# Spijkervet/Context-Aware-Sequential-Recommendation

Hardware: AMD Instinct MI355X
Metric: user-sequences/sec (fwd+bwd) (higher is better)
Workload: dtype f32 (bf16x3 split MFMA in attention); 1 GPU; ml-1m-shaped synthetic (6040 users, 3416 items), cast_1 maxlen=200 hidden_units=50 num_blocks=2 num_heads=1 dropout=0.20, batch 128/GPU (global 128), fwd+bwd+dense TF-Adam per step; parallelism=dp1, hip_graph=True, steps_per_graph_launch=4, attn_precision=bf16x3

## Files before the change

### context-aware-sequential-recommendation_amd/csrc/cr_adam.hip

```cpp
#include <math.h>
#include <stdlib.h>
#include <string.h>

#include "cr_common.hpp"
#include "cr_tgrad.hpp"

int tg_unit_grid(const cr_tgrad_desc* d);

#define ADAM_COLS 256
#define ADAM_WAVES 16
typedef float f4a __attribute__((ext_vector_type(4), aligned(4)));
__device__ __forceinline__ float slab_sum256(const float* slabs, int n_slabs, int n_dense, int j0, float (*part)[ADAM_COLS]) {
    const int lane = threadIdx.x & 63, w = threadIdx.x >> 6;
    const int j = j0 + 4 * lane;
    f4a acc = (f4a){0.f, 0.f, 0.f, 0.f};
    if (j + 3 < n_dense) {
        for (int s0 = w; s0 < n_slabs; s0 += 16 * ADAM_WAVES) {
            f4a v[16];
            int cnt = 0;
#pragma unroll
            for (int u = 0; u < 16; ++u)
                if (s0 + ADAM_WAVES * u < n_slabs) { v[u] = *reinterpret_cast<const f4a*>(slabs + (size_t)(s0 + ADAM_WAVES * u) * n_dense + j); cnt = u + 1; }
#pragma unroll
            for (int u = 0; u < 16; ++u)
// ... 1 lines not shown
        }
    } else {
        for (int s = w; s < n_slabs; s += ADAM_WAVES)
            for (int u = 0; u < 4; ++u)
                if (j + u < n_dense) acc[u] += slabs[(size_t)s * n_dense + j + u];
    }
    part[w][4 * lane + 0] = acc.x; part[w][4 * lane + 1] = acc.y; part[w][4 * lane + 2] = acc.z; part[w][4 * lane + 3] = acc.w;
    __syncthreads();
    float g = 0.0f;
    if (threadIdx.x < ADAM_COLS) {
#pragma unroll
        for (int k = 0; k < ADAM_WAVES; ++k) g += part[k][threadIdx.x];
    }
    return g;
}

template <bool STREAM, int LPR, int VEC>
__global__ __launch_bounds__(64 * ADAM_WAVES) void k_adam(cr_adam_desc d, cr_tgrad_desc g, int nb_dense, int nb_lazy, int nb_units, int nb_ring) {
    __shared__ float part_s[ADAM_WAVES * ADAM_COLS + 4];
    float (*part)[ADAM_COLS] = reinterpret_cast<float (*)[ADAM_COLS]>(part_s);
    constexpr bool TG = LPR > 0;
    cr_kernarg_touch<sizeof(cr_adam_desc) + (TG ? sizeof(cr_tgrad_desc) : 0)>();
    const uint32_t t = d.step_snapshot ? *d.step_snapshot : *reinterpret_cast<const uint32_t*>(d.state + 4);
    const int bid = (int)blockIdx.x;
    if (bid >= (int)gridDim.x - nb_ring) {
        constexpr int NT = 64 * ADAM_WAVES;
        const long long n_copy = d.ids_copy_elems ? d.ids_copy_elems : d.ids_slot_elems;
        const int32_t* src1 = d.ids_ring + (long long)((t + 1u) % (uint32_t)d.ids_ring_slots) * d.ids_slot_elems;
        const long long first = (long long)(bid - ((int)gridDim.x - nb_ring)) * NT + threadIdx.x, stride = (long long)nb_ring * NT;
        if ((d.ids_slot_elems & 3) == 0 && (n_copy & 3) == 0 && (((uintptr_t)d.ids_ring | (uintptr_t)d.ids_dst) & 15) == 0) {
            const int4* src = reinterpret_cast<const int4*>(src1);
            int4* dst = reinterpret_cast<int4*>(d.ids_dst);
            for (long long i = first; i < (n_copy >> 2); i += stride) dst[i] = src[i];
        } else {
            for (long long i = first; i < n_copy; i += stride) d.ids_dst[i] = src1[i];
        }
        return;
    }
    const float* st = d.stats ? d.stats : d.state;
    const float n = st[2];
    float inv_n = 0.0f, lr_t = 0.0f;
    auto scalars = [&]() {
        inv_n = n > 0.0f ? 1.0f / n : 0.0f;
        const float b1t = powf(d.beta1, (float)t), b2t = powf(d.beta2, (float)t);
        lr_t = d.lr * sqrtf(1.0f - b2t) / (1.0f - b1t);
    };
    auto update = [&](long long i, float g) {
        g *= inv_n;
        if (i < d.n_l2) g = fmaf(d.l2, d.p[i], g);
        const float m = d.beta1 * d.m[i] + (1.0f - d.beta1) * g;
        const float v = d.beta2 * d.v[i] + (1.0f - d.beta2) * g * g;
        d.m[i] = m;
        d.v[i] = v;
        d.p[i] -= lr_t * m / (sqrtf(v) + d.eps);
    };
    if (bid < nb_dense) {
        const int j0 = bid * ADAM_COLS;
// ... 171 lines not shown
        }
        for (; q < n4; q += stride) update4(q);
        if (tb == 0) {
            for (long long i = first + threadIdx.x; i < a0; i += NT) {
                const float g = d.table_grad[i];
                d.table_grad[i] = 0.0f;
                update(i, g);
            }
            for (long long i = a0 + 4 * n4 + threadIdx.x; i < d.n_table; i += NT) {
                const float g = d.table_grad[i];
                d.table_grad[i] = 0.0f;
                update(i, g);
            }
        }
    }
    if (bid == 0 && threadIdx.x == 0) {
        d.state[5] = (n > 0.0f ? st[0] / n : 0.0f) + (d.n_l2 > 0 ? d.state[7] : 0.0f);
        d.state[6] = n > 0.0f ? st[1] / n : 0.0f;
        if (d.step_snapshot) {
            d.state[0] = 0.0f; d.state[1] = 0.0f; d.state[2] = 0.0f; d.state[3] = 0.0f;
            *reinterpret_cast<uint32_t*>(d.state + 4) = t + 1u;
        }
    }
}

extern "C" int cr_adam_step(const cr_adam_desc* d, void* stream) {
    CR_REQUIRE(d && d->p && d->m && d->v && d->state, "cr_adam_step: NULL pointer");
    CR_REQUIRE(d->n_table >= 0 && d->n_dense >= 0 && d->n_table + d->n_dense > 0, "cr_adam_step: bad sizes");
    CR_REQUIRE(d->n_table == 0 || d->table_grad || d->tg, "cr_adam_step: table_grad is NULL");
    CR_REQUIRE(d->n_dense == 0 || (d->dense_slabs && d->n_slabs > 0), "cr_adam_step: dense_slabs missing");
    CR_REQUIRE(d->step_snapshot == nullptr || d->stats != nullptr, "cr_adam_step: step_snapshot needs stats (a copy of the sums that does not alias state[0..2])");
    const int nb_dense = cr_ceil_div(d->n_dense, ADAM_COLS);
    int nb_lazy = 0;
    long long n_swept = d->n_table;
    if (d->lazy_ids) {
        CR_REQUIRE(d->lazy_flags && d->n_lazy_ids > 0 && d->lazy_rows > 0 && d->lazy_D > 0 &&
                   (long long)d->lazy_rows * d->lazy_D <= d->n_table, "cr_adam_step: bad lazy-row arguments");
        nb_lazy = cr_ceil_div(d->n_lazy_ids, ADAM_WAVES * 8);
        if (nb_lazy > 4096) nb_lazy = 4096;
        n_swept = d->n_table - (long long)d->lazy_rows * d->lazy_D;
    }
    constexpr int NT = 64 * ADAM_WAVES;
    const long long groups = n_swept / 4 + 1;
    int nb_table = (int)((groups + NT - 1) / NT > 1024 ? 1024 : (groups + NT - 1) / NT);
    if (nb_table < 1) nb_table = 1;
    int nb_ring = 0;
// ... 83 lines not shown
```

### context-aware-sequential-recommendation_amd/csrc/cr_rbwd.hpp

```cpp
#pragma once
#include "cr_rlayout.hpp"

#define SB_WAVES 8
#define SB_NT (64 * SB_WAVES)
#define SB_TPR 7
#define SB_IMG (SB_TPR * 16 * 64)


template <int NWT, int NT, bool SPLIT>
__device__ __forceinline__ void w_put_perm(__bf16* Wi, WRegs<NWT, NT>& r, int D, W3_PARAMS) {
    constexpr int WST = SPLIT ? 2 * ST_WIMG : ST_WIMG;
#pragma unroll
    for (int u = 0; u < (NWT * 512 + NT - 1) / NT; ++u) {
        const int item = tid_now() + NT * u;
        if (item < NWT * 512) {
            const int wi = item >> 9, k = (item & 511) >> 3, ch = item & 7;
            const bool rok = k < D;
            const bool fix = item_fix(rok, k == D - 1, 8 * ch, D);
            item_mask(r.v[u], 8 * ch, D, rok, fix);
            if (__builtin_expect(fix, 0)) {
                const WSrc s = w_pick(wi, W3_ARGS);
                item_refill(r.v[u], s.p + (size_t)k * s.ld + s.c0, 8 * ch, D);
            }
            bf8 h, l;
// ... 209 lines not shown
            const float sg = cr_row16_sum(ag[ct][r]), sb = cr_row16_sum(ab[ct][r]);
            if (li == 0) {
                part[wave * 64 + 16 * ct + 4 * lg + r] = sg;
                part[(SB_WAVES + wave) * 64 + 16 * ct + 4 * lg + r] = sb;
            }
        }
    __syncthreads();
    for (int c = threadIdx.x; c < D; c += SB_NT) {
        float g = 0.0f, b = 0.0f;
#pragma unroll
        for (int w = 0; w < SB_WAVES; ++w) { g += part[w * 64 + c]; b += part[(SB_WAVES + w) * 64 + c]; }
        dg[c] = g;
        db[c] = b;
    }
}
```

### context-aware-sequential-recommendation_amd/csrc/cr_stack.hip

```cpp
#include <math.h>
#include <stdlib.h>
#include <string.h>

#include "cr_attn_common.hpp"
#include "cr_bf16.hpp"

#define ST_WAVES 8
#define ST_THREADS (64 * ST_WAVES)
#define ST_NVEC 11

struct StackBlk { cr_block_desc bd; cr_attn_desc ad; };
struct StackArgs {
    int nb, T16, nkt;
    unsigned char ptile[2][8];
    float isd_log2e, invT;
    const float* lnf_g; const float* lnf_b; float* out; int ld_out, col_out;
    unsigned long long* ts;
    int gather;
    cr_embed_desc e;
    StackBlk blk[CR_STACK_MAX_BLOCKS];
    cr_head_desc hd;
    cr_ln_bwd_desc hl;
};

// ... 398 lines not shown
            for (int ct = 0; ct < 4; ++ct)
#pragma unroll
                for (int r = 0; r < 4; ++r) {
                    float v = acc[ct][r] + bias[ct][r];
                    v *= drop_factor_x(d2, e1 + d2.key + (uint32_t)(16 * ct + r) * CR_PHI);
                    acc[ct][r] = (v + fin[ct][r]) * msk;
                }
            r_store(d.y, mo, acc, rok, dcx);
            if (i == 0) SK_TS(8 + 10 * b);
            if (last && a.out) {
                r_layernorm<false>(fin, acc, vec + 9 * 64, vec + 10 * 64, dcx);
                r_store(a.out + a.col_out, (u32)m * (u32)(4 * a.ld_out), fin, rok, dcx);
            }
            if (HEAD && last) {
                const StackArgs& ah = stack_args_again();
                f32x4 ep[4], en[4], pr[4];
                r_finish(ep, hrp, dcx);
                r_finish(en, hrn, dcx);
#pragma unroll
                for (int ct = 0; ct < 4; ++ct) pr[ct] = ep[ct] * fin[ct];
                const float pl = r_rowsum(pr);
#pragma unroll
                for (int ct = 0; ct < 4; ++ct) pr[ct] = en[ct] * fin[ct];
                const float nl = r_rowsum(pr);
                const float ist = (rok && hpid != 0) ? 1.0f : 0.0f;
                const float sp = 1.0f / (1.0f + expf(-pl)), sn = 1.0f / (1.0f + expf(-nl));
                const float dpl = -ist * sp * (1.0f - sp) / (sp + 1e-24f);
                const float dnl = ist * sn * (1.0f - sn) / (1.0f - sn + 1e-24f);
                float h_loss = 0.0f, h_auc = 0.0f, h_n = 0.0f;
                if (lg == 0 && rok) {
// ... 10 lines not shown
                    const float wl = wave_sum(h_loss), wa = wave_sum(h_auc), wn = wave_sum(h_n);
                    float* red = hpart + 2 * NW * 64;
                    if (ln == 0) { red[wave] = wl; red[NW + wave] = wa; red[2 * NW + wave] = wn; }
                }
                f32x4 dyh[4], dxh[4];
#pragma unroll
                for (int ct = 0; ct < 4; ++ct)
#pragma unroll
                    for (int r = 0; r < 4; ++r) dyh[ct][r] = fmaf(dpl, ep[ct][r], dnl * en[ct][r]);
                if (ah.hd.d_seq_emb) r_store(ah.hd.d_seq_emb, (u32)m * (u32)(4 * ah.hd.ldd), dyh, rok, dcx);
                f32x4 hag[4], hab[4];
#pragma unroll
                for (int ct = 0; ct < 4; ++ct) { hag[ct] = (f32x4){0.f, 0.f, 0.f, 0.f}; hab[ct] = hag[ct]; }
                r_ln_bwd(dxh, acc, dyh, vec + 9 * 64, hag, hab, dcx);
                r_store(ah.hl.dx, (u32)m * (u32)(4 * ah.hl.lddx), dxh, rok, dcx);
#pragma unroll
                for (int ct = 0; ct < 4; ++ct)
#pragma unroll
                    for (int r = 0; r < 4; ++r) {
                        const float sg = cr_row16_sum(hag[ct][r]), sb = cr_row16_sum(hab[ct][r]);
                        if (li == 0) {
                            hpart[wave * 64 + 16 * ct + 4 * lg + r] = sg;
                            hpart[(NW + wave) * 64 + 16 * ct + 4 * lg + r] = sb;
                        }
                    }
            }
        }
        SK_TS(10 + 10 * b);
        if (!last) {
            const cr_block_desc& dn = a.blk[b + 1].bd;
            w_issue<2, NT>(wa, D, dn.wqkv, 3 * D, D, dn.wqkv, 3 * D, 2 * D, dn.wqkv, 3 * D, 2 * D);
            vec_issue<NT>(vv, dn, a, D);
            issue_x(dn.x, max(tile_a(0), 0), 0, false);
        }
        if (!last) __syncthreads();
    }
    if (HEAD) {
        const StackArgs& ah = stack_args_again();
        float* red = hpart + 2 * NW * 64;
        if (nB == 0) {
            hpart[wave * 64 + (threadIdx.x & 63)] = 0.0f;
            hpart[(NW + wave) * 64 + (threadIdx.x & 63)] = 0.0f;
            if ((threadIdx.x & 63) == 0) { red[wave] = 0.0f; red[NW + wave] = 0.0f; red[2 * NW + wave] = 0.0f; }
        }
        __syncthreads();
        const unsigned slab = blockIdx.y * gridDim.x + blockIdx.x;
        if ((int)threadIdx.x < D) {
            float g = 0.0f, bsum = 0.0f;
#pragma unroll
            for (int w = 0; w < NW; ++w) { g += hpart[w * 64 + threadIdx.x]; bsum += hpart[(NW + w) * 64 + threadIdx.x]; }
            ah.hl.dgamma[(size_t)slab * ah.hl.slab_stride + threadIdx.x] = g;
            ah.hl.dbeta[(size_t)slab * ah.hl.slab_stride + threadIdx.x] = bsum;
        }
        if (threadIdx.x < 3) {
            float v = 0.0f;
            for (int w = 0; w < NW; ++w) v += red[NW * threadIdx.x + w];
            if (v != 0.0f) atomicAdd(ah.hd.state + threadIdx.x, v);
        }
        head_snapshot_at(ah.hd.state, gridDim.x * gridDim.y, reinterpret_cast<int*>(red + 3 * NW));
    }
    SK_TS(63);
}

static size_t stack_lds_bytes(int T16, bool split, bool head = false, int nkt_template = 0) {
    const size_t kb = head ? (size_t)16 * nkt_template * 4 : (size_t)T16 * 4;
    return (size_t)T16 * 64 * 2 * (split ? 4 : 2) + (size_t)3 * ST_WIMG * 2 * (split ? 2 : 1) + (size_t)ST_NVEC * 64 * 4 + kb
           + (head ? (size_t)(2 * ST_WAVES * 64 + 3 * ST_WAVES + 4) * 4 : 0);
}

static const char* stack_unsupported(const cr_stack_desc* s) {
    if (!s || !s->blocks || !s->attn) return "NULL description";
    if (s->n_blocks < 1 || s->n_blocks > CR_STACK_MAX_BLOCKS) return "1..4 blocks";
    const cr_block_desc& b0 = s->blocks[0];
    const cr_attn_desc& a0 = s->attn[0];
// ... 185 lines not shown
```

### context-aware-sequential-recommendation_amd/csrc/cr_stack_bwd1.hip

```cpp
#include <math.h>
#include <stdlib.h>
#include <string.h>
#include <type_traits>
#include <mutex>

#include "cr_rbwd.hpp"

#define B1_DRAIN() asm volatile("s_waitcnt vmcnt(0)" ::: "memory")
#define B1_NT_WS true
#define B1_ROWS 224
#define B1_FSTR (B1_ROWS * 64)

#define DS_EXACT(DS) ((DS) > 0 ? ((DS) & 255) : (DS))
#define DS_D(DS, run) ((DS) > 0 ? ((DS) & 255) : (run))
#define B1_NKT(DS, a) ((DS) > 255 ? (((DS) >> 8) & 255) : (a).nkt)
#define B1_T(DS, a) ((DS) > 65535 ? ((DS) >> 16) : (a).T)
#undef D_NF
#define D_NF(DS) ((DS) > 0 ? ((DS) & 255) / 16 : ((DS) < 0 ? -(DS) - 1 : -1))

struct B1Args {
    cr_block_bwd_desc bd;
    cr_attn_desc ad;
    cr_embed_bwd_desc sc;
    cr_ln_bwd_desc ln;
// ... 49 lines not shown
template <bool BIAS = false>
__device__ __forceinline__ void b1_wstore(float* dst, int ldw, float* bias_dst, const f32x4 (&acc)[2], const f32x4 (&accb)[2], int D, int it, int jt0, bool add) {
    const int lane = threadIdx.x & 63, li = lane & 15, lg = lane >> 4;
#pragma unroll
    for (int j = 0; j < 2; ++j) {
        const int col = 16 * (jt0 + j) + li;
#pragma unroll
        for (int r = 0; r < 4; ++r) {
            const int k = 16 * it + 4 * lg + r;
            if (col < D && (BIAS ? k < D : k <= D)) {
                float* p = (k < D) ? dst + (size_t)k * ldw + col : bias_dst + col;
                __builtin_nontemporal_store(add ? *p + acc[j][r] : acc[j][r], p);
            }
        }
        if (BIAS && it == 0 && lg == 0 && col < D) bias_dst[col] = add ? bias_dst[col] + accb[j][0] : accb[j][0];
    }
}
__device__ __forceinline__ void b1_ln_fold(float* part, const f32x4 (&ag)[4], const f32x4 (&ab)[4]) {
    const int lane = lane_now(), wave = __builtin_amdgcn_readfirstlane(threadIdx.x >> 6), lg = lane >> 4;
    float u[16];
#pragma unroll
    for (int ct = 0; ct < 4; ++ct)
#pragma unroll
        for (int r = 0; r < 4; ++r) {
            float x = ag[ct][r];
            asm volatile("s_nop 1\n\t"
                         "v_add_f32_dpp %0, %0, %0 row_mirror row_mask:0xf bank_mask:0x3\n\t"
                         "v_add_f32_dpp %0, %1, %1 row_mirror row_mask:0xf bank_mask:0xc"
                         : "+v"(x) : "v"(ab[ct][r]));
            u[4 * ct + r] = x;
        }
#pragma unroll
    for (int j = 0; j < 8; ++j)
        asm volatile("s_nop 1\n\t"
                     "v_add_f32_dpp %0, %0, %0 row_half_mirror row_mask:0xf bank_mask:0x5\n\t"
                     "v_add_f32_dpp %0, %1, %1 row_half_mirror row_mask:0xf bank_mask:0xa"
                     : "+v"(u[j]) : "v"(u[8 + j]));
    const bool b1 = (lane & 2) != 0, b0 = (lane & 1) != 0;
    float w[4], z[2];
#pragma unroll
    for (int j = 0; j < 4; ++j) {
        const float keep = b1 ? u[4 + j] : u[j], send = b1 ? u[j] : u[4 + j];
        w[j] = keep + __int_as_float(__builtin_amdgcn_update_dpp(0, __float_as_int(send), 0x1B, 0xF, 0xF, false));
    }
#pragma unroll
    for (int j = 0; j < 2; ++j) {
        const float keep = b0 ? w[2 + j] : w[j], send = b0 ? w[j] : w[2 + j];
        z[j] = keep + __int_as_float(__builtin_amdgcn_update_dpp(0, __float_as_int(send), 0xB1, 0xF, 0xF, false));
    }
    const int col = 16 * (((lane >> 2) & 1) * 2 + ((lane >> 1) & 1)) + 4 * lg + 2 * (lane & 1);
    float* dst = part + ((lane & 8) ? SB_WAVES * 64 : 0) + wave * 64 + col;
    *reinterpret_cast<float2*>(dst) = make_float2(z[0], z[1]);
}
template <int NSET = 1>
__device__ __forceinline__ void b1_ln_flush(const float* part, float* dg, float* db, int D, bool add) {
    for (int c = threadIdx.x; c < D; c += SB_NT) {
        float g = 0.0f, b = 0.0f;
#pragma unroll
        for (int s = 0; s < NSET; ++s)
#pragma unroll
            for (int w = 0; w < SB_WAVES; ++w) { g += part[(2 * s * SB_WAVES + w) * 64 + c]; b += part[((2 * s + 1) * SB_WAVES + w) * 64 + c]; }
        dg[c] = add ? dg[c] + g : g;
        db[c] = add ? db[c] + b : b;
    }
}

struct B1Steps { uint32_t ffn2, attn, emb; };
struct B1Acc { f32x4 aw1[2], aw2[2], aw1b[2], aw2b[2], ag[4], ab[4], agF[4], abF[4]; };

template <bool SPLIT, int DS, bool QSIDE, int HD, class F>
__device__ __forceinline__ void b1_phase1(const B1Args& a, unsigned char* smem, int n, B1Acc& A, B1Steps& steps, F&& before_last_products) {
    constexpr bool BIAS = DS_EXACT(DS) == 64;
    constexpr bool LATE_Q = !QSIDE && (HD == 2 || DS_EXACT(DS) > 50 || DS <= 0);
    typedef B1Lds<SPLIT> L;
    const cr_block_bwd_desc& bd = a.bd;
    const cr_block_desc& d = bd.f;
    __bf16* Im = reinterpret_cast<__bf16*>(smem);
    __bf16* Wi = Im + L::W_OFF;
// ... 634 lines not shown
        r_store<B1_NT_WS>(const_cast<float*>(ar.bd.dqkv), mo, dq, rok, dcx);
        f32x4 dqin[4];
        {
            bf8 gh[2], gl[2];
            r_split<SPLIT>(dq, gh, gl);
            r_gemm_t<SPLIT, false>(dqin, Wi, Wi + ST_WIMG, gh, gl);
#pragma unroll
            for (int ct = 0; ct < 4; ++ct) dqin[ct] += dO[ct];
        }
        f32x4 x[4], dxl[4], ag[4], ab[4];
#pragma unroll
        for (int ct = 0; ct < 4; ++ct) { ag[ct] = (f32x4){0.f, 0.f, 0.f, 0.f}; ab[ct] = ag[ct]; }
        r_finish(x, rx, dcx);
        if (ti == 0 && (int)((tpk >> 5) & 31u) < B1_NKT(DS, a)) issue_tile((int)((tpk >> 5) & 31u));
        r_ln_bwd(dxl, x, dqin, gam, ag, ab, dcx);
        b1_ln_fold(part + ti * (2 * SB_WAVES * 64), ag, ab);
        if (ar.bd.dx_accumulate) {
            f32x4 old[4];
            r_finish(old, rdx, dcx);
#pragma unroll
            for (int ct = 0; ct < 4; ++ct) dxl[ct] += old[ct];
        }
        if (ar.scatter) {
            b1_scatter_prep(ar, dxl, m, rok, D, steps.emb);
            r_store(ar.sbuf, mo, dxl, rok, dcx);
        } else {
            r_store(ar.bd.dx, mo, dxl, rok, dcx);
        }
    }
    B1_TS(4);
    __builtin_amdgcn_s_setprio(0);
// ... 24 lines not shown
        f32x4 qin[4], dQ[4];
        r_finish(qin, rq1, dcx);
        plant_one(qin, D);
        img_put<SPLIT>(Im, Im + B1_FSTR, 16 * tt1, qin);
        r_finish(dQ, rg1, dcx);
        img_put<SPLIT>(Gm, Gm + B1_FSTR, 16 * tt1, dQ);
    }
    B1Small small;
    if (a.scatter && a.small) b1_small_issue<D_NF(DS)>(small, a, a.sbuf, n, D);
    __syncthreads();
    B1_TS(16);
    wgrad_accum<SPLIT, BIAS, 2 * SB_TPR>(awq, nob, Im, Im + B1_FSTR, Gm, Gm + B1_FSTR, B1_NKT(DS, a), it, jt0);
    B1_TS(17);
    const size_t so = (size_t)blockIdx.x * bd.slab_stride;
    b1_wstore<BIAS>(bd.g_wqkv + so, 3 * D, bd.g_bqkv + so, awq, nob, D, it, jt0, add);
    b1_ln_flush<2>(part, bd.g_ln1_g + so, bd.g_ln1_b + so, D, add);
    B1_TS(18);
    if (a.scatter && a.small) b1_small_table<SPLIT, D_NF(DS)>(a, smem, reinterpret_cast<int*>(part), small, n, D, add);
    else if (a.scatter) b1_scatter_rows(a, a.sbuf, n, D);
    B1_TS(5);
    (void)MD;
}

template <bool SPLIT, int DS, int HD>
__device__ __forceinline__ void b1_k_side(const B1Args& a, unsigned char* smem, int n, bool add, B1Acc& A, const B1Steps& steps) {
    constexpr bool BIAS = DS_EXACT(DS) == 64;
    typedef B1Lds<SPLIT> L;
    const cr_block_bwd_desc& bd = a.bd;
    const cr_block_desc& bk = bd.f;
    const cr_attn_desc& d = a.ad;
    __bf16* Im = reinterpret_cast<__bf16*>(smem);
// ... 9 lines not shown
    const size_t MD = (size_t)M * D;
    float* dKg = const_cast<float*>(bd.dqkv) + MD;
    float* dVg = const_cast<float*>(bd.dqkv) + 2 * MD;
    typedef float f4s __attribute__((ext_vector_type(4), aligned(4)));
    const DropCtx dc = drop_ctx(d.drop, steps.attn);
    {
        WRegs<2, SB_NT> w;
        w_issue<2, SB_NT>(w, D, bk.wqkv, 3 * D, D, bk.wqkv, 3 * D, 2 * D, bk.wqkv, 3 * D, 2 * D);
        const int t = threadIdx.x, tc = min(t, T - 1);
        f4s st[HD];
#pragma unroll
        for (int h = 0; h < HD; ++h) st[h] = *reinterpret_cast<const f4s*>(d.row_stats + ((size_t)h * d.B * T + base_row + tc) * 4);
        const float qv = d.q_valid[base_row + tc];
        {
            float* part = fl + L::PART; float* partF = fl + L::PARTF;
            b1_ln_fold(part, A.ag, A.ab);
            if (a.has_ln) b1_ln_fold(partF, A.agF, A.abF);
            __syncthreads();
            const size_t so = (size_t)blockIdx.x * bd.slab_stride;
            b1_ln_flush(part, bd.g_ln2_g + so, bd.g_ln2_b + so, D, add);
            if (a.has_ln) b1_ln_flush(partF, a.ln.dgamma + so, a.ln.dbeta + so, D, add);
        }
        w_put_perm<2, SB_NT, SPLIT>(Wi, w, D, bk.wqkv, 3 * D, D, bk.wqkv, 3 * D, 2 * D, bk.wqkv, 3 * D, 2 * D);
        const float flag = t < T ? st[0].z : 2.0f;
        const bool normal = flag == 0.0f;
        if (t < T16 + ((B1_NKT(DS, a) & 1) ? 16 : 0)) {
#pragma unroll
            for (int h = 0; h < HD; ++h) {
                smx[h * B1_ROWS + t] = normal ? st[h].x - __log2f(st[h].y) : 1e30f;
                if (!normal || t >= T16) sdel[h * B1_ROWS + t] = 0.0f;
            }
            suni[t] = (flag == 1.0f) ? a.invT : 0.0f;
            sqv[t] = t < T ? qv * dc.scale : 0.0f;
        }
        if ((t & ~63) < T16) {
            const bool live = t < T16;
// ... 460 lines not shown
```

### context-aware-sequential-recommendation_amd/engine.py

```python
import ctypes as C
import math
import os
import zlib

import numpy as np
import torch

from . import lib as L
from . import ops as O

ATTN_PRECISIONS = {"f32": L.PREC_F32, "bf16x3": L.PREC_BF16X3, "bf16": L.PREC_BF16}
DEFAULT_ATTN_PRECISION = "bf16x3"
LOSSES = ("bce", "ce")
ALL_LOSSES = LOSSES + ("sampled_ce", "gbce")
SOFTMAX_LOSSES = ("ce", "sampled_ce", "gbce")
SAMPLED_LOSSES = ("sampled_ce", "gbce")
CE_PROPOSALS = ("uniform", "popularity")

MODELS = ["cast_1", "cast_2", "cast_3", "cast_4", "cast_5", "cast_6", "cast_7", "cast_8", "cast_9",
          "sasrec", "sasrec_static"]


def site_id(name):
    return zlib.crc32(name.encode()) & 0xFFFFFF
# ... 238 lines not shown
                      else O.sampled_ce_workspace_bytes(self.M, self.ce_negatives, self.D) if self.loss == "sampled_ce"
                      else O.gbce_workspace_bytes(self.M, self.ce_negatives, self.D))
                self._ce_ws = torch.empty(nb, dtype=torch.uint8, device=self.dev)
            if self.loss in SAMPLED_LOSSES:
                self.samples = torch.zeros(self.ce_negatives, dtype=torch.int32, device=self.dev)
            if self.ce_proposal == "popularity":
                self.item_cdf = torch.zeros(itemnum + 1, dtype=torch.int32, device=self.dev)
                self.item_logq = torch.zeros(itemnum + 1, **f32)
                self._have_item_weights = False
        self.drop = O.Drop(hp.dropout_rate if training else 0.0, self.seed, self.state, row_offset)
        self.batch_global = self.B if batch_global is None else batch_global
        self.want_attn = want_attn
        self.attn_weights = None
        self._bufs, self._keep = {}, []
        self.fwd, self.bwd = [], []
        self._bwd_factories = []
        self._grad_written = set()
        i32 = dict(dtype=torch.int32, device=self.dev)
        self.ID_KEYS = ("seq", "pos", "neg", "time", "hours", "days")
        ng, ent = C.c_int(0), C.c_int(0)
        self.use_index = bool(training and not self.lazy_adam and self.loss == "bce" and os.environ.get("CASTREC_NO_INDEX") != "1"
                              and L.lib.cr_tgrad_geometry(self.D, C.byref(ng), C.byref(ent)))
        self.ids_words = 6 * self.M
        self.index_off = (self.ids_words + 3) // 4 * 4
        self.index_lay, self._ixb = None, None
        if self.use_index:
            self.index_lay = L.IndexLayout()
            t_pos = self.T if "pos_emb" in self.layout.entries else 0
            L.check(L.lib.cr_batch_index_layout(self.M, itemnum + 1, t_pos, ng.value, ent.value, C.byref(self.index_lay)), "cr_batch_index_layout")
            self._ixb = L.lib.cr_index_builder_create(self.M, itemnum + 1, t_pos, ng.value, ent.value)
# ... 622 lines not shown
        if rec is not None:
            x, pname = rec
            dx = self._grad_of(x)
            assert self._acc(id(dx)) == 0
            self._ln_claimed.add(seq_emb.data_ptr())
            d = L.HeadDesc(seq_emb.data_ptr(), seq_emb.shape[1], self._pptr("item_emb"), self.ids["pos"].data_ptr(),
                           self.ids["neg"].data_ptr(), M, D, self.itemnum + 1, self.state.data_ptr(), None, 0,
                           None if self.use_index else self._gptr("item_emb"), None, None, self._head_coef())
            n = L.LnBwdDesc(x.data_ptr(), D, self._pptr(pname + ".gamma"), None, 0, dx.data_ptr(), D, 0,
                            self._gptr(pname + ".gamma"), self._gptr(pname + ".beta"), self.Gs.shape[1], self.n_slabs, M, D, 1e-8)
            last = self.fwd[-1] if self.fwd else None
            if (self.use_index and last is not None and last[0] == "cr_stack_fwd" and os.environ.get("CASTREC_NO_HEAD_FUSION") != "1"
                    and last[2][0]._obj.out == seq_emb.data_ptr()
                    and L.lib.cr_stack_fwd_head_supported(last[2][0], C.byref(d), C.byref(n))):
                self._keep += [d, n]
                self.fwd[-1] = ("cr_stack_fwd_head", L.lib.cr_stack_fwd_head, (last[2][0], C.byref(d), C.byref(n)))
                self._block_slab_range(pname + ".gamma", pname + ".beta", 2 * self.B)
                return
            self._call(self.fwd, "cr_head_fwd_bwd_ln", C.byref(d), C.byref(n))
            return
        ds = self._grad_of(seq_emb)
        self._grad_written.add(id(ds))
        d = L.HeadDesc(seq_emb.data_ptr(), seq_emb.shape[1], self._pptr("item_emb"), self.ids["pos"].data_ptr(),
                       self.ids["neg"].data_ptr(), M, D, self.itemnum + 1, self.state.data_ptr(), ds.data_ptr(), ds.shape[1],
                       None if self.use_index else self._gptr("item_emb"), None, None, self._head_coef())
        self._call(self.fwd, "cr_head_fwd_bwd", C.byref(d))

    def _head_coef(self):
        if not self.use_index:
            return None
# ... 119 lines not shown
            if self.n_wslabs < self.n_slabs:
                for a, b in self._wgrad_ranges:
                    per[a:b] = self.n_wslabs
            for a, b, c in self._block_bwd_ranges:
                per[a:b] = c
            if lay.n_dense and int(per.min()) < self.n_slabs:
                nb = (lay.n_dense + 255) // 256
                pad = np.zeros(nb * 256, np.int32)
                pad[:lay.n_dense] = per
                cnt = pad.reshape(nb, 256).max(1).astype(np.int32)
                self.slab_counts = torch.from_numpy(cnt).to(self.dev)
                counts = self.slab_counts.data_ptr()
            ad = L.AdamDesc(self.P.data_ptr(), self.Mom.data_ptr(), self.Vel.data_ptr(), self.Gt.data_ptr(), self.Gs.data_ptr(),
                            lay.n_table, lay.n_dense, self.n_slabs, float(self.hp.lr), 0.9, 0.98, 1e-8, self.state.data_ptr(),
                            snap, tsnap, l2, n_l2, *lazy, counts)
            self._tgd, self._tgrad = None, None
            if self.use_index:
                assert self._tg_rows is not None, "occurrence index: no gradient-row buffer for the item table's seq lookup"
                rows, rows2, ld_rows, scale = self._tg_rows
                se = self.seq_emb
                self._tgd = L.TgradDesc(self.batch_buf.data_ptr() + 4 * self.index_off, None, 0, 0, 0, self.state.data_ptr() + 4 * 4,
                                        self.index_lay, rows.data_ptr(), rows2.data_ptr() if rows2 is not None else None, ld_rows, scale,
                                        se.data_ptr(), se.shape[1], self._head_coef(), self.D, self._tg_part.data_ptr(), self._tg_tickets.data_ptr())
                ad.tg = C.pointer(self._tgd)
                self._tgrad = ("cr_table_grad", L.lib.cr_table_grad, (C.byref(self._tgd), self.Gt.data_ptr()))
            self._adam = ("cr_adam_step", L.lib.cr_adam_step, (C.byref(ad),))
            ad1 = L.AdamDesc(self.P.data_ptr(), self.Mom.data_ptr(), self.Vel.data_ptr(), self.Gt.data_ptr(),
                             self.Gflat.data_ptr() + 4 * lay.n_table, lay.n_table, lay.n_dense, 1, float(self.hp.lr), 0.9, 0.98,
                             1e-8, self.state.data_ptr(), self.Gflat.data_ptr() + 4 * lay.n_total, tsnap, l2, n_l2, *lazy, None)
            self._adam_flat = ("cr_adam_step", L.lib.cr_adam_step, (C.byref(ad1),))
# ... 83 lines not shown
                raise RuntimeError("castrec %s failed (%d): %s" % (name, rc, L.lib.cr_last_error().decode()))

    def launch_step(self, apply=True, between=None, capturing=False):
        s = torch.cuda.current_stream().cuda_stream
        if self.training and not capturing:
            self._need_item_weights()
        self._run(self.fwd, s)
        if self.training:
            self._run(self.bwd, s)
            if between is not None:
                between()
            if apply:
                self._run(([self._l2] if self._l2 else []) + [self._adam], s)
                if self._id_ring is not None and self.lazy_adam:
                    self._run([self._ring_next], s)

    def use_id_ring(self, ring):
        ads = [self._adam[2][0]._obj, self._adam_flat[2][0]._obj]
        if ring is None:
            self._id_ring = None
            for ad in ads:
                ad.ids_ring, ad.ids_ring_slots, ad.ids_slot_elems, ad.ids_dst, ad.ids_copy_elems = None, 0, 0, None, 0
            if self._tgd is not None:
                self._tgd.ring, self._tgd.ring_slots, self._tgd.slot_words, self._tgd.index_off = None, 0, 0, 0
            return
        assert ring.dtype == torch.int32 and ring.is_cuda and ring.is_contiguous(), ring.shape
        assert int(np.prod(ring.shape[1:])) == self.slot_words, \
            "ring slots of %s words, the engine's slots have %d (pack_slot: 6 x %d ids%s)" % (tuple(ring.shape[1:]), self.slot_words, self.M, " + the occurrence index" if self.use_index else "")
        self._id_ring = ring
        if self.lazy_adam:
# ... 90 lines not shown
        marks = [j for j in range(k, last + 1) if j % self._feed_every == 0]
        if G > 1 and last not in marks:
            marks.append(last)
        if marks:
            ev = torch.cuda.Event()
            ev.record(cur)
            for j in marks:
                self._feed_done[j] = ev
            for old in [j for j in self._feed_done if j < last - n]:
                del self._feed_done[old]
        self._feed_have -= G
        return G

    def launch_backward_to_flat(self):
        s = torch.cuda.current_stream().cuda_stream
        self._run(self.fwd, s)
        self._run(self.bwd, s)
        self._run(([self._tgrad] if self._tgrad else []) + [self._reduce], s)

    def launch_adam_from_flat(self):
        self._run(([self._l2] if self._l2 else []) + [self._adam_flat], torch.cuda.current_stream().cuda_stream)

    def capture_dp_phases(self):
        s0 = torch.cuda.current_stream()
        side = torch.cuda.Stream()
        side.wait_stream(s0)
        k = self.bwd_table_done
        progs = [self.fwd + self.bwd[:k] + ([self._tgrad] if self._tgrad else []), self.bwd[k:] + [self._reduce],
                 ([self._l2] if self._l2 else []) + [self._adam_flat]]
        graphs = []
        with torch.cuda.stream(side):
            for prog in progs:
                g = O.Graph()
                g.begin()
                self._run(prog, torch.cuda.current_stream().cuda_stream)
                g.end()
                graphs.append(g)
        s0.wait_stream(side)
        self.dp_graphs, self.dp_progs, self._graph_stream = graphs, progs, side
        return graphs

    def capture(self, dp=False, n_steps=1):
        side = torch.cuda.Stream()
# ... 103 lines not shown
```

### context-aware-sequential-recommendation_amd/lib.py

```python
import ctypes as C
import os

import torch

from . import PKG_DIR

LIB_PATH = os.path.join(PKG_DIR, "libcastrec_tl.so" if os.environ.get("CASTREC_TIMELINE") == "1" else "libcastrec.so")
if os.environ.get("CASTREC_LIB"):
    LIB_PATH = os.path.abspath(os.environ["CASTREC_LIB"])
if not os.path.exists(LIB_PATH):
    raise ImportError("castrec_amd: native library %s not found -- build it with "
                      "`python -m castrec_amd.build` (needs hipcc, gfx950). There is no CPU fallback." % LIB_PATH)
_lib = C.CDLL(LIB_PATH)

c_f = C.c_float
c_i = C.c_int
c_u32 = C.c_uint32
c_p = C.c_void_p

CR_MAX_BATCH = 4
CR_STATE_FLOATS = 16
CR_SCE_MAX_SAMPLES = 16384
CR_SCE_SITE = 0x5CE00000
CR_GBCE_SITE = 0x6BCE0000
# ... 74 lines not shown


class BlockTailDesc(C.Structure):
    _fields_ = [("kind", c_i), ("next", C.POINTER(BlockDesc)), ("lnf_gamma", c_p), ("lnf_beta", c_p), ("out", c_p),
                ("ld_out", c_i), ("col_out", c_i)]


class StackDesc(C.Structure):
    _fields_ = [("n_blocks", c_i), ("blocks", C.POINTER(BlockDesc)), ("attn", C.POINTER(AttnDesc)), ("lnf_gamma", c_p),
                ("lnf_beta", c_p), ("out", c_p), ("ld_out", c_i), ("col_out", c_i), ("embed", C.POINTER(EmbedDesc))]


class HeadDesc(C.Structure):
    _fields_ = [("seq_emb", c_p), ("ld", c_i), ("table", c_p), ("pos", c_p), ("neg", c_p),
                ("M", c_i), ("D", c_i), ("V", c_i), ("state", c_p), ("d_seq_emb", c_p), ("ldd", c_i),
                ("table_grad", c_p), ("pos_logits", c_p), ("neg_logits", c_p), ("coef_out", c_p)]


class IndexLayout(C.Structure):
    _fields_ = [("M", c_i), ("V", c_i), ("T_pos", c_i), ("ng", c_i), ("ent", c_i), ("cap_blocks", c_i), ("cap_occ", c_i), ("bitmap_words", c_i),
                ("off_recs", C.c_int64), ("total_words", C.c_int64)]


class TgradDesc(C.Structure):
    _fields_ = [("index", c_p), ("ring", c_p), ("ring_slots", c_i), ("slot_words", C.c_int64), ("index_off", C.c_int64), ("step", c_p),
                ("lay", IndexLayout), ("rows", c_p), ("rows2", c_p), ("ld_rows", c_i), ("scale", c_f), ("seq_emb", c_p), ("ld_emb", c_i),
                ("coef", c_p), ("D", c_i), ("part_rows", c_p), ("tickets", c_p)]


class AdamDesc(C.Structure):
    _fields_ = [("p", c_p), ("m", c_p), ("v", c_p), ("table_grad", c_p), ("dense_slabs", c_p),
                ("n_table", C.c_int64), ("n_dense", c_i), ("n_slabs", c_i), ("lr", c_f), ("beta1", c_f),
                ("beta2", c_f), ("eps", c_f), ("state", c_p), ("stats", c_p), ("step_snapshot", c_p), ("l2", c_f), ("n_l2", C.c_int64),
                ("lazy_ids", c_p), ("n_lazy_ids", c_i), ("lazy_rows", c_i), ("lazy_D", c_i), ("lazy_flags", c_p), ("slab_counts", c_p),
                ("ids_ring", c_p), ("ids_ring_slots", c_i), ("ids_slot_elems", C.c_int64), ("ids_dst", c_p),
                ("ids_copy_elems", C.c_int64), ("tg", C.POINTER(TgradDesc))]


CR_TOPK_MAX = 128


class TopkDesc(C.Structure):
    _fields_ = [("query", c_p), ("ld", c_i), ("table", c_p), ("V", c_i), ("D", c_i), ("B", c_i), ("K", c_i), ("precision", c_i),
                ("excl_off", c_p), ("excl_ids", c_p), ("targets", c_p), ("top_ids", c_p), ("top_scores", c_p), ("rank", c_p),
                ("workspace", c_p), ("workspace_bytes", C.c_size_t)]


class SoftmaxCeDesc(C.Structure):
    _fields_ = [("seq_emb", c_p), ("ld", c_i), ("table", c_p), ("pos", c_p), ("neg", c_p), ("M", c_i), ("D", c_i), ("V", c_i),
                ("precision", c_i), ("state", c_p), ("d_seq_emb", c_p), ("ldd", c_i), ("table_grad", c_p), ("lse_out", c_p),
                ("workspace", c_p), ("workspace_bytes", C.c_size_t)]
# ... 114 lines not shown
```

### include/castrec.h

```cpp
#ifndef CASTREC_H
#define CASTREC_H

#include <stddef.h>
#include <stdint.h>

#ifdef __cplusplus
extern "C" {
#endif

#define CR_OK 0
#define CR_ERR_INVALID (-1)
#define CR_ERR_UNSUPPORTED (-2)
#define CR_ERR_HIP (-3)

#define CR_MAX_BATCH 4
#define CR_STATE_FLOATS 16

int cr_version(void);
const char* cr_last_error(void);

typedef struct {
    float rate;
    uint32_t site;
    uint32_t seed;
// ... 207 lines not shown
int cr_wide_ln_ffn_bwd(const cr_block_bwd_desc* d, float* g2, float* g1, int heads, int precision, void* stream);
int cr_wide_ln_qkv_bwd(const cr_block_bwd_desc* d, int precision, void* stream);

int cr_block_ln_qkv_bwd_scatter(const cr_block_bwd_desc* bd, const cr_embed_bwd_desc* sc, void* stream);

typedef struct {
    const float* seq_emb; int ld;
    const float* table;
    const int32_t* pos; const int32_t* neg;
    int M, D, V;
    float* state;
    float* d_seq_emb; int ldd;
    float* table_grad;
    float* pos_logits; float* neg_logits;
    float* coef_out;
} cr_head_desc;
int cr_head_fwd_bwd(const cr_head_desc* d, void* stream);

int cr_head_fwd_bwd_ln(const cr_head_desc* d, const cr_ln_bwd_desc* n, void* stream);

int cr_stack_fwd_head_supported(const cr_stack_desc* d, const cr_head_desc* h, const cr_ln_bwd_desc* n);
int cr_stack_fwd_head(const cr_stack_desc* d, const cr_head_desc* h, const cr_ln_bwd_desc* n, void* stream);

int cr_test_logits(const float* seq_emb, int ld, const float* table, const int32_t* cand,
                   int B, int T, int D, int V, int n_cand, float* logits, void* stream);

#define CR_TOPK_MAX 128
typedef struct cr_topk_desc cr_topk_desc;
struct cr_topk_desc {
    const float* query; int ld;
// ... 113 lines not shown
    float* table_grad;
    const float* dense_slabs;
    int64_t n_table;
    int n_dense, n_slabs;
    float lr, beta1, beta2, eps;
    float* state;
    const float* stats;
    const uint32_t* step_snapshot;
    float l2; int64_t n_l2;
    const int32_t* lazy_ids; int n_lazy_ids, lazy_rows, lazy_D;
    uint32_t* lazy_flags;
    const int32_t* slab_counts;
    const int32_t* ids_ring; int ids_ring_slots; int64_t ids_slot_elems; int32_t* ids_dst;
    int64_t ids_copy_elems;
    const cr_tgrad_desc* tg;
} cr_adam_desc;
int cr_adam_step(const cr_adam_desc* d, void* stream);

int cr_l2_penalty(const float* p, int64_t n, float scale, float* state, void* stream);

int cr_reduce_slabs(const float* dense_slabs, int n_slabs, int n_dense, float* out,
                    const float* state, float* stats_out, const int32_t* slab_counts , void* stream);

int cr_rows_pack(float* table, const int32_t* ids, int n, int D, int V, uint32_t* flags, const uint32_t* tag, float* packed,
                 int zero_rows, void* stream);
int cr_rows_add(float* table, const float* packed, int n, int D, int V, void* stream);

int cr_graph_begin(void* stream);
int cr_graph_end(void* stream, void** graph_exec_out);
int cr_graph_launch(void* graph_exec, void* stream);
// ... 16 lines not shown
```

Baseline: 409,700 sequences/s.

## Replace head loss atomics with per-block stat partials reduced inside Adam

The fused stack+head kernel now writes each block's loss, AUC and count partials to a per-slab buffer instead of issuing atomicAdds on shared state and running the last-block snapshot. The Adam kernel reduces these partials with wave-level reductions to get the normalizer and the reported metrics. The head's LayerNorm gamma/beta partial reduction is also switched to the shared DPP-based fold routine, now moved from the backward file into the common header. This removes atomic contention and the snapshot serialization at the end of the head. In exchange Adam does extra reads, and a separate descriptor path is kept for non-graph runs.

```diff
diff --git a/context-aware-sequential-recommendation_amd/csrc/cr_adam.hip b/context-aware-sequential-recommendation_amd/csrc/cr_adam.hip
--- a/context-aware-sequential-recommendation_amd/csrc/cr_adam.hip
+++ b/context-aware-sequential-recommendation_amd/csrc/cr_adam.hip
@@ -39,6 +39,13 @@
     }
     return g;
 }
+
+__device__ __forceinline__ float lanes_total(float v) {
+    v = cr_row16_sum(v);
+    auto row = [&](int l) { return __int_as_float(__builtin_amdgcn_readlane(__float_as_int(v), l)); };
+    return __int_as_float(__builtin_amdgcn_readfirstlane(__float_as_int(((row(0) + row(16)) + row(32)) + row(48))));
+}
+#define ADAM_SP_PRE 4
 
 template <bool STREAM, int LPR, int VEC>
 __global__ __launch_bounds__(64 * ADAM_WAVES) void k_adam(cr_adam_desc d, cr_tgrad_desc g, int nb_dense, int nb_lazy, int nb_units, int nb_ring) {
@@ -63,9 +70,22 @@
         return;
     }
     const float* st = d.stats ? d.stats : d.state;
-    const float n = st[2];
+    const int sp_lane = threadIdx.x & 63;
+    float sp[ADAM_SP_PRE], sp_n = 0.0f;
+#pragma unroll
+    for (int u = 0; u < ADAM_SP_PRE; ++u) {
+        sp[u] = 0.0f;
+        if (d.stat_parts && sp_lane + 64 * u < d.n_stat_parts) sp[u] = d.stat_parts[4 * (sp_lane + 64 * u) + 2];
+    }
+    float n = d.stat_parts ? 0.0f : st[2];
     float inv_n = 0.0f, lr_t = 0.0f;
     auto scalars = [&]() {
+        if (d.stat_parts) {
+#pragma unroll
+            for (int u = 0; u < ADAM_SP_PRE; ++u) sp_n += sp[u];
+            for (int i = sp_lane + 64 * ADAM_SP_PRE; i < d.n_stat_parts; i += 64) sp_n += d.stat_parts[4 * i + 2];
+            n = lanes_total(sp_n);
+        }
         inv_n = n > 0.0f ? 1.0f / n : 0.0f;
         const float b1t = powf(d.beta1, (float)t), b2t = powf(d.beta2, (float)t);
         lr_t = d.lr * sqrtf(1.0f - b2t) / (1.0f - b1t);
@@ -267,9 +287,17 @@
             }
         }
     }
+    float loss_sum = 0.0f, auc_sum = 0.0f;
+    if (bid == 0 && threadIdx.x < 64) {
+        if (d.stat_parts) {
+            f4a acc = (f4a){0.f, 0.f, 0.f, 0.f};
+            for (int i = sp_lane; i < d.n_stat_parts; i += 64) acc += *reinterpret_cast<const f4a*>(d.stat_parts + 4 * i);
+            loss_sum = lanes_total(acc.x); auc_sum = lanes_total(acc.y);
+        } else { loss_sum = st[0]; auc_sum = st[1]; }
+    }
     if (bid == 0 && threadIdx.x == 0) {
-        d.state[5] = (n > 0.0f ? st[0] / n : 0.0f) + (d.n_l2 > 0 ? d.state[7] : 0.0f);
-        d.state[6] = n > 0.0f ? st[1] / n : 0.0f;
+        d.state[5] = (n > 0.0f ? loss_sum / n : 0.0f) + (d.n_l2 > 0 ? d.state[7] : 0.0f);
+        d.state[6] = n > 0.0f ? auc_sum / n : 0.0f;
         if (d.step_snapshot) {
             d.state[0] = 0.0f; d.state[1] = 0.0f; d.state[2] = 0.0f; d.state[3] = 0.0f;
             *reinterpret_cast<uint32_t*>(d.state + 4) = t + 1u;
@@ -283,6 +311,8 @@
     CR_REQUIRE(d->n_table == 0 || d->table_grad || d->tg, "cr_adam_step: table_grad is NULL");
     CR_REQUIRE(d->n_dense == 0 || (d->dense_slabs && d->n_slabs > 0), "cr_adam_step: dense_slabs missing");
     CR_REQUIRE(d->step_snapshot == nullptr || d->stats != nullptr, "cr_adam_step: step_snapshot needs stats (a copy of the sums that does not alias state[0..2])");
+    CR_REQUIRE(d->stat_parts == nullptr || (d->n_stat_parts > 0 && d->n_stat_parts <= 4096 && ((uintptr_t)d->stat_parts & 15) == 0),
+               "cr_adam_step: stat_parts: 1..4096 entries of 16 bytes, 16-byte aligned");
     const int nb_dense = cr_ceil_div(d->n_dense, ADAM_COLS);
     int nb_lazy = 0;
     long long n_swept = d->n_table;
diff --git a/context-aware-sequential-recommendation_amd/csrc/cr_rbwd.hpp b/context-aware-sequential-recommendation_amd/csrc/cr_rbwd.hpp
--- a/context-aware-sequential-recommendation_amd/csrc/cr_rbwd.hpp
+++ b/context-aware-sequential-recommendation_amd/csrc/cr_rbwd.hpp
@@ -247,3 +247,52 @@
         db[c] = b;
     }
 }
+
+__device__ __forceinline__ void r_ln_fold(float* part, const f32x4 (&ag)[4], const f32x4 (&ab)[4]) {
+    const int lane = lane_now(), wave = __builtin_amdgcn_readfirstlane(threadIdx.x >> 6), lg = lane >> 4;
+    float u[16];
+#pragma unroll
+    for (int ct = 0; ct < 4; ++ct)
+#pragma unroll
+        for (int r = 0; r < 4; ++r) {
+            float x = ag[ct][r];
+            asm volatile("s_nop 1\n\t"
+                         "v_add_f32_dpp %0, %0, %0 row_mirror row_mask:0xf bank_mask:0x3\n\t"
+                         "v_add_f32_dpp %0, %1, %1 row_mirror row_mask:0xf bank_mask:0xc"
+                         : "+v"(x) : "v"(ab[ct][r]));
+            u[4 * ct + r] = x;
+        }
+#pragma unroll
+    for (int j = 0; j < 8; ++j)
+        asm volatile("s_nop 1\n\t"
+                     "v_add_f32_dpp %0, %0, %0 row_half_mirror row_mask:0xf bank_mask:0x5\n\t"
+                     "v_add_f32_dpp %0, %1, %1 row_half_mirror row_mask:0xf bank_mask:0xa"
+                     : "+v"(u[j]) : "v"(u[8 + j]));
+    const bool b1 = (lane & 2) != 0, b0 = (lane & 1) != 0;
+    float w[4], z[2];
+#pragma unroll
+    for (int j = 0; j < 4; ++j) {
+        const float keep = b1 ? u[4 + j] : u[j], send = b1 ? u[j] : u[4 + j];
+        w[j] = keep + __int_as_float(__builtin_amdgcn_update_dpp(0, __float_as_int(send), 0x1B, 0xF, 0xF, false));
+    }
+#pragma unroll
+    for (int j = 0; j < 2; ++j) {
+        const float keep = b0 ? w[2 + j] : w[j], send = b0 ? w[j] : w[2 + j];
+        z[j] = keep + __int_as_float(__builtin_amdgcn_update_dpp(0, __float_as_int(send), 0xB1, 0xF, 0xF, false));
+    }
+    const int col = 16 * (((lane >> 2) & 1) * 2 + ((lane >> 1) & 1)) + 4 * lg + 2 * (lane & 1);
+    float* dst = part + ((lane & 8) ? SB_WAVES * 64 : 0) + wave * 64 + col;
+    *reinterpret_cast<float2*>(dst) = make_float2(z[0], z[1]);
+}
+template <int NSET = 1>
+__device__ __forceinline__ void r_ln_flush(const float* part, float* dg, float* db, int D, bool add) {
+    for (int c = threadIdx.x; c < D; c += SB_NT) {
+        float g = 0.0f, b = 0.0f;
+#pragma unroll
+        for (int s = 0; s < NSET; ++s)
+#pragma unroll
+            for (int w = 0; w < SB_WAVES; ++w) { g += part[(2 * s * SB_WAVES + w) * 64 + c]; b += part[((2 * s + 1) * SB_WAVES + w) * 64 + c]; }
+        dg[c] = add ? dg[c] + g : g;
+        db[c] = add ? db[c] + b : b;
+    }
+}
diff --git a/context-aware-sequential-recommendation_amd/csrc/cr_stack.hip b/context-aware-sequential-recommendation_amd/csrc/cr_stack.hip
--- a/context-aware-sequential-recommendation_amd/csrc/cr_stack.hip
+++ b/context-aware-sequential-recommendation_amd/csrc/cr_stack.hip
@@ -436,6 +436,7 @@
             }
             if (HEAD && last) {
                 const StackArgs& ah = stack_args_again();
+                SK_TS(50);
                 f32x4 ep[4], en[4], pr[4];
                 r_finish(ep, hrp, dcx);
                 r_finish(en, hrn, dcx);
@@ -476,16 +477,10 @@
                 for (int ct = 0; ct < 4; ++ct) { hag[ct] = (f32x4){0.f, 0.f, 0.f, 0.f}; hab[ct] = hag[ct]; }
                 r_ln_bwd(dxh, acc, dyh, vec + 9 * 64, hag, hab, dcx);
                 r_store(ah.hl.dx, (u32)m * (u32)(4 * ah.hl.lddx), dxh, rok, dcx);
-#pragma unroll
-                for (int ct = 0; ct < 4; ++ct)
-#pragma unroll
-                    for (int r = 0; r < 4; ++r) {
-                        const float sg = cr_row16_sum(hag[ct][r]), sb = cr_row16_sum(hab[ct][r]);
-                        if (li == 0) {
-                            hpart[wave * 64 + 16 * ct + 4 * lg + r] = sg;
-                            hpart[(NW + wave) * 64 + 16 * ct + 4 * lg + r] = sb;
-                        }
-                    }
+                static_assert(NW == SB_WAVES, "r_ln_fold's slots: [2][SB_WAVES][64]");
+                SK_TS(51);
+                r_ln_fold(hpart, hag, hab);
+                SK_TS(52);
             }
         }
         SK_TS(10 + 10 * b);
@@ -506,6 +501,7 @@
             if ((threadIdx.x & 63) == 0) { red[wave] = 0.0f; red[NW + wave] = 0.0f; red[2 * NW + wave] = 0.0f; }
         }
         __syncthreads();
+        SK_TS(53);
         const unsigned slab = blockIdx.y * gridDim.x + blockIdx.x;
         if ((int)threadIdx.x < D) {
             float g = 0.0f, bsum = 0.0f;
@@ -514,12 +510,24 @@
             ah.hl.dgamma[(size_t)slab * ah.hl.slab_stride + threadIdx.x] = g;
             ah.hl.dbeta[(size_t)slab * ah.hl.slab_stride + threadIdx.x] = bsum;
         }
-        if (threadIdx.x < 3) {
-            float v = 0.0f;
-            for (int w = 0; w < NW; ++w) v += red[NW * threadIdx.x + w];
-            if (v != 0.0f) atomicAdd(ah.hd.state + threadIdx.x, v);
-        }
-        head_snapshot_at(ah.hd.state, gridDim.x * gridDim.y, reinterpret_cast<int*>(red + 3 * NW));
+        if (ah.hd.parts) {
+            const unsigned pt = threadIdx.x - 64u;
+            if (pt < 4u) {
+                float v = 0.0f;
+                if (pt < 3u)
+                    for (int w = 0; w < NW; ++w) v += red[NW * pt + w];
+                ah.hd.parts[4 * (size_t)slab + pt] = v;
+            }
+            if (slab == 0 && threadIdx.x == 128) *reinterpret_cast<unsigned*>(ah.hd.state + 11) = *reinterpret_cast<const unsigned*>(ah.hd.state + 4);
+        } else {
+            if (threadIdx.x < 3) {
+                float v = 0.0f;
+                for (int w = 0; w < NW; ++w) v += red[NW * threadIdx.x + w];
+                if (v != 0.0f) atomicAdd(ah.hd.state + threadIdx.x, v);
+            }
+            head_snapshot_at(ah.hd.state, gridDim.x * gridDim.y, reinterpret_cast<int*>(red + 3 * NW));
+        }
+        SK_TS(54);
     }
     SK_TS(63);
 }
diff --git a/context-aware-sequential-recommendation_amd/csrc/cr_stack_bwd1.hip b/context-aware-sequential-recommendation_amd/csrc/cr_stack_bwd1.hip
--- a/context-aware-sequential-recommendation_amd/csrc/cr_stack_bwd1.hip
+++ b/context-aware-sequential-recommendation_amd/csrc/cr_stack_bwd1.hip
@@ -87,54 +87,6 @@
             }
         }
         if (BIAS && it == 0 && lg == 0 && col < D) bias_dst[col] = add ? bias_dst[col] + accb[j][0] : accb[j][0];
-    }
-}
-__device__ __forceinline__ void b1_ln_fold(float* part, const f32x4 (&ag)[4], const f32x4 (&ab)[4]) {
-    const int lane = lane_now(), wave = __builtin_amdgcn_readfirstlane(threadIdx.x >> 6), lg = lane >> 4;
-    float u[16];
-#pragma unroll
-    for (int ct = 0; ct < 4; ++ct)
-#pragma unroll
-        for (int r = 0; r < 4; ++r) {
-            float x = ag[ct][r];
-            asm volatile("s_nop 1\n\t"
-                         "v_add_f32_dpp %0, %0, %0 row_mirror row_mask:0xf bank_mask:0x3\n\t"
-                         "v_add_f32_dpp %0, %1, %1 row_mirror row_mask:0xf bank_mask:0xc"
-                         : "+v"(x) : "v"(ab[ct][r]));
-            u[4 * ct + r] = x;
-        }
-#pragma unroll
-    for (int j = 0; j < 8; ++j)
-        asm volatile("s_nop 1\n\t"
-                     "v_add_f32_dpp %0, %0, %0 row_half_mirror row_mask:0xf bank_mask:0x5\n\t"
-                     "v_add_f32_dpp %0, %1, %1 row_half_mirror row_mask:0xf bank_mask:0xa"
-                     : "+v"(u[j]) : "v"(u[8 + j]));
-    const bool b1 = (lane & 2) != 0, b0 = (lane & 1) != 0;
-    float w[4], z[2];
-#pragma unroll
-    for (int j = 0; j < 4; ++j) {
-        const float keep = b1 ? u[4 + j] : u[j], send = b1 ? u[j] : u[4 + j];
-        w[j] = keep + __int_as_float(__builtin_amdgcn_update_dpp(0, __float_as_int(send), 0x1B, 0xF, 0xF, false));
-    }
-#pragma unroll
-    for (int j = 0; j < 2; ++j) {
-        const float keep = b0 ? w[2 + j] : w[j], send = b0 ? w[j] : w[2 + j];
-        z[j] = keep + __int_as_float(__builtin_amdgcn_update_dpp(0, __float_as_int(send), 0xB1, 0xF, 0xF, false));
-    }
-    const int col = 16 * (((lane >> 2) & 1) * 2 + ((lane >> 1) & 1)) + 4 * lg + 2 * (lane & 1);
-    float* dst = part + ((lane & 8) ? SB_WAVES * 64 : 0) + wave * 64 + col;
-    *reinterpret_cast<float2*>(dst) = make_float2(z[0], z[1]);
-}
-template <int NSET = 1>
-__device__ __forceinline__ void b1_ln_flush(const float* part, float* dg, float* db, int D, bool add) {
-    for (int c = threadIdx.x; c < D; c += SB_NT) {
-        float g = 0.0f, b = 0.0f;
-#pragma unroll
-        for (int s = 0; s < NSET; ++s)
-#pragma unroll
-            for (int w = 0; w < SB_WAVES; ++w) { g += part[(2 * s * SB_WAVES + w) * 64 + c]; b += part[((2 * s + 1) * SB_WAVES + w) * 64 + c]; }
-        dg[c] = add ? dg[c] + g : g;
-        db[c] = add ? db[c] + b : b;
     }
 }
 
@@ -799,7 +751,7 @@
         r_finish(x, rx, dcx);
         if (ti == 0 && (int)((tpk >> 5) & 31u) < B1_NKT(DS, a)) issue_tile((int)((tpk >> 5) & 31u));
         r_ln_bwd(dxl, x, dqin, gam, ag, ab, dcx);
-        b1_ln_fold(part + ti * (2 * SB_WAVES * 64), ag, ab);
+        r_ln_fold(part + ti * (2 * SB_WAVES * 64), ag, ab);
         if (ar.bd.dx_accumulate) {
             f32x4 old[4];
             r_finish(old, rdx, dcx);
@@ -854,7 +806,7 @@
     B1_TS(17);
     const size_t so = (size_t)blockIdx.x * bd.slab_stride;
     b1_wstore<BIAS>(bd.g_wqkv + so, 3 * D, bd.g_bqkv + so, awq, nob, D, it, jt0, add);
-    b1_ln_flush<2>(part, bd.g_ln1_g + so, bd.g_ln1_b + so, D, add);
+    r_ln_flush<2>(part, bd.g_ln1_g + so, bd.g_ln1_b + so, D, add);
     B1_TS(18);
     if (a.scatter && a.small) b1_small_table<SPLIT, D_NF(DS)>(a, smem, reinterpret_cast<int*>(part), small, n, D, add);
     else if (a.scatter) b1_scatter_rows(a, a.sbuf, n, D);
@@ -894,12 +846,12 @@
         const float qv = d.q_valid[base_row + tc];
         {
             float* part = fl + L::PART; float* partF = fl + L::PARTF;
-            b1_ln_fold(part, A.ag, A.ab);
-            if (a.has_ln) b1_ln_fold(partF, A.agF, A.abF);
+            r_ln_fold(part, A.ag, A.ab);
+            if (a.has_ln) r_ln_fold(partF, A.agF, A.abF);
             __syncthreads();
             const size_t so = (size_t)blockIdx.x * bd.slab_stride;
-            b1_ln_flush(part, bd.g_ln2_g + so, bd.g_ln2_b + so, D, add);
-            if (a.has_ln) b1_ln_flush(partF, a.ln.dgamma + so, a.ln.dbeta + so, D, add);
+            r_ln_flush(part, bd.g_ln2_g + so, bd.g_ln2_b + so, D, add);
+            if (a.has_ln) r_ln_flush(partF, a.ln.dgamma + so, a.ln.dbeta + so, D, add);
         }
         w_put_perm<2, SB_NT, SPLIT>(Wi, w, D, bk.wqkv, 3 * D, D, bk.wqkv, 3 * D, 2 * D, bk.wqkv, 3 * D, 2 * D);
         const float flag = t < T ? st[0].z : 2.0f;
diff --git a/context-aware-sequential-recommendation_amd/engine.py b/context-aware-sequential-recommendation_amd/engine.py
--- a/context-aware-sequential-recommendation_amd/engine.py
+++ b/context-aware-sequential-recommendation_amd/engine.py
@@ -276,6 +276,7 @@
         self.attn_weights = None
         self._bufs, self._keep = {}, []
         self.fwd, self.bwd = [], []
+        self.head_parts, self._head_dp = None, None
         self._bwd_factories = []
         self._grad_written = set()
         i32 = dict(dtype=torch.int32, device=self.dev)
@@ -928,6 +929,12 @@
                     and last[2][0]._obj.out == seq_emb.data_ptr()
                     and L.lib.cr_stack_fwd_head_supported(last[2][0], C.byref(d), C.byref(n))):
                 self._keep += [d, n]
+                if os.environ.get("CASTREC_HEAD_ATOMICS") != "1":
+                    d_old = L.HeadDesc.from_buffer_copy(d)
+                    self._keep.append(d_old)
+                    self.head_parts = torch.zeros(2 * self.B, 4, dtype=torch.float32, device=self.dev)
+                    d.parts = self.head_parts.data_ptr()
+                    self._head_dp = (len(self.fwd) - 1, ("cr_stack_fwd_head", L.lib.cr_stack_fwd_head, (last[2][0], C.byref(d_old), C.byref(n))))
                 self.fwd[-1] = ("cr_stack_fwd_head", L.lib.cr_stack_fwd_head, (last[2][0], C.byref(d), C.byref(n)))
                 self._block_slab_range(pname + ".gamma", pname + ".beta", 2 * self.B)
                 return
@@ -1077,6 +1084,8 @@
             ad = L.AdamDesc(self.P.data_ptr(), self.Mom.data_ptr(), self.Vel.data_ptr(), self.Gt.data_ptr(), self.Gs.data_ptr(),
                             lay.n_table, lay.n_dense, self.n_slabs, float(self.hp.lr), 0.9, 0.98, 1e-8, self.state.data_ptr(),
                             snap, tsnap, l2, n_l2, *lazy, counts)
+            if self.head_parts is not None:
+                ad.stat_parts, ad.n_stat_parts = self.head_parts.data_ptr(), int(self.head_parts.shape[0])
             self._tgd, self._tgrad = None, None
             if self.use_index:
                 assert self._tg_rows is not None, "occurrence index: no gradient-row buffer for the item table's seq lookup"
@@ -1190,6 +1199,16 @@
                 self._run(([self._l2] if self._l2 else []) + [self._adam], s)
                 if self._id_ring is not None and self.lazy_adam:
                     self._run([self._ring_next], s)
+            elif self.head_parts is not None and not capturing:
+                tot = self.head_parts.double().sum(0)[:3].float()
+                self.state[0:3] = tot
+                self.state[8:11] = tot
+
+    def _fwd_dp(self):
+        if self._head_dp is None:
+            return self.fwd
+        i, entry = self._head_dp
+        return self.fwd[:i] + [entry] + self.fwd[i + 1:]
 
     def use_id_ring(self, ring):
         ads = [self._adam[2][0]._obj, self._adam_flat[2][0]._obj]
@@ -1310,7 +1329,7 @@
 
     def launch_backward_to_flat(self):
         s = torch.cuda.current_stream().cuda_stream
-        self._run(self.fwd, s)
+        self._run(self._fwd_dp(), s)
         self._run(self.bwd, s)
         self._run(([self._tgrad] if self._tgrad else []) + [self._reduce], s)
 
@@ -1322,7 +1341,7 @@
         side = torch.cuda.Stream()
         side.wait_stream(s0)
         k = self.bwd_table_done
-        progs = [self.fwd + self.bwd[:k] + ([self._tgrad] if self._tgrad else []), self.bwd[k:] + [self._reduce],
+        progs = [self._fwd_dp() + self.bwd[:k] + ([self._tgrad] if self._tgrad else []), self.bwd[k:] + [self._reduce],
                  ([self._l2] if self._l2 else []) + [self._adam_flat]]
         graphs = []
         with torch.cuda.stream(side):
diff --git a/context-aware-sequential-recommendation_amd/lib.py b/context-aware-sequential-recommendation_amd/lib.py
--- a/context-aware-sequential-recommendation_amd/lib.py
+++ b/context-aware-sequential-recommendation_amd/lib.py
@@ -112,7 +112,7 @@
 class HeadDesc(C.Structure):
     _fields_ = [("seq_emb", c_p), ("ld", c_i), ("table", c_p), ("pos", c_p), ("neg", c_p),
                 ("M", c_i), ("D", c_i), ("V", c_i), ("state", c_p), ("d_seq_emb", c_p), ("ldd", c_i),
-                ("table_grad", c_p), ("pos_logits", c_p), ("neg_logits", c_p), ("coef_out", c_p)]
+                ("table_grad", c_p), ("pos_logits", c_p), ("neg_logits", c_p), ("coef_out", c_p), ("parts", c_p)]
 
 
 class IndexLayout(C.Structure):
@@ -132,7 +132,7 @@
                 ("beta2", c_f), ("eps", c_f), ("state", c_p), ("stats", c_p), ("step_snapshot", c_p), ("l2", c_f), ("n_l2", C.c_int64),
                 ("lazy_ids", c_p), ("n_lazy_ids", c_i), ("lazy_rows", c_i), ("lazy_D", c_i), ("lazy_flags", c_p), ("slab_counts", c_p),
                 ("ids_ring", c_p), ("ids_ring_slots", c_i), ("ids_slot_elems", C.c_int64), ("ids_dst", c_p),
-                ("ids_copy_elems", C.c_int64), ("tg", C.POINTER(TgradDesc))]
+                ("ids_copy_elems", C.c_int64), ("tg", C.POINTER(TgradDesc)), ("stat_parts", c_p), ("n_stat_parts", c_i)]
 
 
 CR_TOPK_MAX = 128
diff --git a/include/castrec.h b/include/castrec.h
--- a/include/castrec.h
+++ b/include/castrec.h
@@ -245,6 +245,7 @@
     float* table_grad;
     float* pos_logits; float* neg_logits;
     float* coef_out;
+    float* parts;
 } cr_head_desc;
 int cr_head_fwd_bwd(const cr_head_desc* d, void* stream);
 
@@ -388,6 +389,7 @@
     const int32_t* ids_ring; int ids_ring_slots; int64_t ids_slot_elems; int32_t* ids_dst;
     int64_t ids_copy_elems;
     const cr_tgrad_desc* tg;
+    const float* stat_parts; int n_stat_parts;
 } cr_adam_desc;
 int cr_adam_step(const cr_adam_desc* d, void* stream);
 
```

Measured after the change: 411,000 sequences/s (median of 6 runs). Within noise of the previous version (+0.3%).
